# okieraised/rs-face-detection

Measured on NVIDIA B200. Metric: frames/s preproc+decode+NMS+align, higher is better.
Workload: dtype u8/f32

## Files before the change

rs_face_detection_b200/csrc/fd_align.cu:

```cuda
#include <algorithm>
#include <cmath>
#include <cstdio>
#include <cstdlib>
#include <vector>
#include <cfloat>
#include <type_traits>
#include "fd_internal.cuh"
#include "fd_estimate.cuh"
#include "fd_resize.cuh"

namespace fd {

struct EstArgs {
    const float *from;
    const float *to;
    const int *count_dev;
    int F;
    EstConst ec;
    double *M12;
    double *M_out;
    uint8_t *ok;
    uint8_t *ok_out;
};

// ... 335 lines not shown
    }
#pragma unroll
    for (int u = 0; u < N; ++u) {
        const int p = p0 + u * WARP_THREADS;
        unsigned lo0, hi0, lo1, hi1;
        extract6(q[u][0], q[u][1], off[u], lo0, hi0);
        extract6(q[u][2], q[u][3], off[u] + pitch, lo1, hi1);
        const unsigned v = blend24(lo0, hi0, lo1, hi1, axy[u] & 31, axy[u] >> 8);
        store_px(band_out, p, v, p < npix, packed);
    }
}

template <int FMT>
__device__ __forceinline__ void warp_round_border(const WarpItem &it, const int2 *__restrict__ dxy, const int2 *__restrict__ xy0, int cw,
                                                  unsigned cw_magic, int p0, int npix, uint8_t *band_out, bool packed) {
    const int p = min(p0, npix - 1);
    const int row = cw_magic ? (int)__umulhi((unsigned)p, cw_magic) : p, x = p - row * cw;
    const int2 d = dxy[x], r0 = xy0[row];
    const int X = (int)((unsigned)r0.x + (unsigned)d.x) >> 5, Y = (int)((unsigned)r0.y + (unsigned)d.y) >> 5;
    const unsigned v = FMT != SRC_BGR ? border_tap_blend_yuv<FMT>(it.data, it.pitch, it.uv, it.v, it.pitch_uv, it.w, it.h, X, Y)
                                      : border_tap_blend(it.data, it.w, it.h, it.pitch, it.lo_lim, it.hi_lim, X, Y);
    store_px(band_out, p0, v, p0 < npix, packed);
}

template <int FMT>
__global__ void __launch_bounds__(WARP_THREADS, 4) warp_kernel(WarpArgs a) {
    constexpr bool NV = FMT != SRC_BGR;
    extern __shared__ int2 wsm[];
    int2 *dxy = wsm;
    int2 *xy0 = dxy + a.cw;
    __shared__ int s_item[2];
    const int tid = threadIdx.x;
    pdl_wait();
    const int F = a.count_dev ? min(*a.count_dev, a.F) : a.F;
    const int n_items = F * a.bands;
    if (tid == 0) s_item[0] = atomicAdd(a.ticket, 1);
    __syncthreads();
    for (int par = 0;; par ^= 1) {
        const int item = s_item[par];
        if (item >= n_items) {
            pdl_trigger();
            break;
        }
        if (tid == 0) s_item[par ^ 1] = atomicAdd(a.ticket, 1);
        const int f = item / a.bands, band_y0 = (item - f * a.bands) * WARP_BAND;
        const int rows = min(WARP_BAND, a.ch - band_y0);
        const int npix = rows * a.cw;
        uint8_t *band_out = a.crops + ((size_t)f * a.ch + band_y0) * a.cw * 3;
        const bool packed = (reinterpret_cast<uintptr_t>(band_out) & 3) == 0 && (npix & 3) == 0;
        const FrameDev fr = a.frames[a.frame_idx ? a.frame_idx[f] : 0];
        if (!a.ok[f]) {
            int rx0 = 0, ry0 = 0;
            const bool valid = warp_fallback_roi(a, f, fr.w, fr.h, &rx0, &ry0);
            if (tid == 0 && band_y0 == 0 && a.mode_out) a.mode_out[f] = valid ? 2 : 0;
            if (valid) {
                const uint8_t *roi = fr.data + (size_t)ry0 * fr.pitch + (size_t)rx0 * 3;
                for (int p = tid; p < npix; p += WARP_THREADS) {
                    const int row = p / a.cw, x = p - row * a.cw;
                    const unsigned v = NV ? resize_pixel24_yuv<FMT>(fr.data, fr.pitch, fr.uv, fr.v_plane(), fr.pitch_uv, rx0, ry0, fr.w - rx0, fr.h - ry0, a.cw,
                                                                    a.ch, x, band_y0 + row)
                                          : resize_pixel24(roi, fr.pitch, fr.w - rx0, fr.h - ry0, a.cw, a.ch, x, band_y0 + row);
                    band_out[3 * p] = (uint8_t)v; band_out[3 * p + 1] = (uint8_t)(v >> 8); band_out[3 * p + 2] = (uint8_t)(v >> 16);
                }
            } else {
                for (int p = tid; p < npix * 3; p += WARP_THREADS) band_out[p] = 0;
            }
            __syncthreads();
            continue;
        }
        if (tid == 0 && band_y0 == 0 && a.mode_out) a.mode_out[f] = 1;
        const double *iM = a.M12 + (size_t)f * 12 + 6;
        const double i0 = iM[0], i1 = iM[1], i2 = iM[2], i3 = iM[3], i4 = iM[4], i5 = iM[5];
        for (int x = tid; x < a.cw; x += WARP_THREADS)
            dxy[x] = make_int2(__double2int_rn(i0 * x * 1024), __double2int_rn(i3 * x * 1024));
        if (tid >= WARP_THREADS - WARP_BAND) {
            const int r = tid - (WARP_THREADS - WARP_BAND), y = band_y0 + min(r, rows - 1);
// ... 88 lines not shown
template <int CW, int N, int FMT>
__device__ __forceinline__ void fixed_rounds_interior_yuv(const uint8_t *__restrict__ yp, unsigned py, const uint8_t *__restrict__ uvp,
                                                          const uint8_t *__restrict__ vp, unsigned puv, int2 d, const int2 *__restrict__ xy,
                                                          unsigned *__restrict__ outw, bool store, unsigned pack_sel) {
    YuvQuad<FMT> q[N];
    int axy[N];
#pragma unroll
    for (int u = 0; u < N; ++u) {
        const int2 r0 = xy[2 * u];
        const int X = (int)((unsigned)r0.x + (unsigned)d.x) >> 5, Y = (int)((unsigned)r0.y + (unsigned)d.y) >> 5;
        axy[u] = (X & 31) | ((Y & 31) << 14);
        yuv_quad_load<FMT>(yp, py, uvp, vp, puv, X >> 5, Y >> 5, q[u]);
    }
#pragma unroll
    for (int u = 0; u < N; ++u) {
        unsigned lo0, hi0, lo1, hi1;
        yuv_quad_taps<FMT>(q[u], lo0, hi0, lo1, hi1);
        const unsigned v = blend24_scaled(lo0, hi0, lo1, hi1, axy[u] & 31, axy[u] >> 8);
        const unsigned nv = __shfl_down_sync(0xffffffffu, v, 1);
        if (store) outw[u * (2 * CW * 3 / 4)] = __byte_perm(v, nv, pack_sel);
    }
}

template <int CW, int CH, int IR, int UN, int FMT>
__global__ void __launch_bounds__(2 * CW) warp_fixed_kernel(WarpArgs a) {
    constexpr bool NV = FMT != SRC_BGR;
    constexpr int T = 2 * CW, ITEMS = CH / IR, ROUNDS = IR / 2;
    static_assert(CH % IR == 0 && IR % 2 == 0 && T % 32 == 0 && (2 * CW * 3) % 4 == 0 && (IR * CW * 3) % 4 == 0, "fixed warp geometry");
    __shared__ int2 xy0[2][IR];
    __shared__ int s_item[2];
    const int tid = threadIdx.x;
    const int r = tid / CW, x = tid - r * CW;
    pdl_wait();
    const int F = a.count_dev ? min(*a.count_dev, a.F) : a.F;
    const int n_items = F * ITEMS;
    long long t_entry = 0, t_prev = 0, t_sum = 0;
    int n_done = 0;
    if (a.dbg && tid == 0) t_entry = warp_now();
    if (tid == 0) s_item[0] = atomicAdd(a.ticket, 1);
    __syncthreads();
    if (a.dbg && tid == 0) { t_prev = warp_now(); a.dbg[blockIdx.x * 8 + 1] = t_prev; }
    for (int par = 0;; par ^= 1) {
        const int item = s_item[par];
        if (a.dbg && tid == 0 && par == 1 && n_done == 1) a.dbg[blockIdx.x * 8 + 2] = warp_now();
        if (a.dbg && tid == 0) { const long long t = warp_now(); if (n_done) t_sum += t - t_prev; t_prev = t; ++n_done; }
        if (item >= n_items) {
            pdl_trigger();
            break;
        }
        if (tid == 0) s_item[par ^ 1] = atomicAdd(a.ticket, 1);
        const int f = item / ITEMS, y0 = (item - f * ITEMS) * IR;
        uint8_t *band_out = a.crops + ((size_t)f * CH + y0) * CW * 3;
        const bool okf = a.ok[f] != 0;
        const FrameDev *frp = a.frames + (a.frame_idx ? a.frame_idx[f] : 0);
        const uint8_t *data = frp->data;
        const int fw = frp->w, fh = frp->h, pitch = frp->pitch;
        const uint8_t *uvp = NV ? frp->uv : nullptr;
        const int pitch_uv = NV ? frp->pitch_uv : 0;
        const uint8_t *vp = nullptr;
        if constexpr (FMT == SRC_PLANAR) vp = frp->v_plane();
        int2 d = make_int2(0, 0);
        bool vote = true;
        if (okf) {
            const double *iM = a.M12 + (size_t)f * 12 + 6;
            const double i0 = iM[0], i3 = iM[3];
            d = make_int2(__double2int_rn(i0 * x * 1024), __double2int_rn(i3 * x * 1024));
            if (tid < IR || tid >= T - 4) {
                const double i1 = iM[1], i2 = iM[2], i4 = iM[4], i5 = iM[5];
                if (tid < IR) {
                    const int y = y0 + tid;
                    xy0[par][tid] = make_int2(__double2int_rn((i1 * y + i2) * 1024) + 16, __double2int_rn((i4 * y + i5) * 1024) + 16);
                } else {
                    const int c = tid - (T - 4), cx = (c & 1) ? CW - 1 : 0, y = y0 + ((c & 2) ? IR - 1 : 0);
                    const long long Xl = (long long)(__double2int_rn((i1 * y + i2) * 1024) + 16) + __double2int_rn(i0 * cx * 1024);
                    const long long Yl = (long long)(__double2int_rn((i4 * y + i5) * 1024) + 16) + __double2int_rn(i3 * cx * 1024);
                    const long long sx = Xl >> 10, sy = Yl >> 10;
                    vote = sx >= 0 && sx + 1 < fw && sy >= 0 && sy + 1 < fh - (NV ? 2 : 1);
                }
            }
        }
        const bool interior = __syncthreads_and(vote) && (NV ? yuv_interior_ok<FMT>(*frp)
                                                                 : (reinterpret_cast<uintptr_t>(data) & 7) == 0 && (pitch & 7) == 0 && pitch >= 16 &&
// ... 103 lines not shown
                    double *M12_dev, double *M_out_dev, uint8_t *ok_dev, uint8_t *ok_out_dev) {
    if (F_cap <= 0) return FD_OK;
    EstArgs a;
    a.from = from_dev;
    a.to = to_dev;
    a.count_dev = count_dev;
    a.F = F_cap;
    FD_TRY(make_est_const(ctx, &a.ec));
    a.M12 = M12_dev;
    a.M_out = M_out_dev;
    a.ok = ok_dev;
    a.ok_out = ok_out_dev;
    estimate_kernel<<<(F_cap * EST_LANES + 127) / 128, 128, 0, ctx->stream>>>(a);
    FD_LAUNCH_CHECK_NAMED(ctx, "estimate_kernel");
    return FD_OK;
}

int invert_launch(fd_ctx *ctx, const double *M_dev, int F, double *M12_dev, uint8_t *ok_dev) {
    if (F <= 0) return FD_OK;
    invert_kernel<<<(F + 127) / 128, 128, 0, ctx->stream>>>(M_dev, F, M12_dev, ok_dev);
    FD_LAUNCH_CHECK(ctx);
    return FD_OK;
}

template <int IR>
static void (*fixed_kernel_for(int fmt))(WarpArgs) {
    return fmt == SRC_NV12 ? warp_fixed_kernel<112, 112, IR, 4, SRC_NV12>
           : fmt == SRC_NV21 ? warp_fixed_kernel<112, 112, IR, 4, SRC_NV21>
           : fmt == SRC_PLANAR ? warp_fixed_kernel<112, 112, IR, 2, SRC_PLANAR> : warp_fixed_kernel<112, 112, IR, 4, SRC_BGR>;
}
static const char *const FIXED_NAMES[4] = {"warp_fixed_kernel", "warp_fixed_kernel_nv12", "warp_fixed_kernel_nv21", "warp_fixed_kernel_i420"};
static const char *const WARP_NAMES[4] = {"warp_kernel", "warp_kernel_nv12", "warp_kernel_nv21", "warp_kernel_i420"};

int warp_launch(fd_ctx *ctx, const FrameDev *frames_dev, const int32_t *frame_idx_dev, const double *M12_dev,
                const uint8_t *ok_dev, const int *count_dev, int F_cap, uint8_t *crops_dev, int cw, int ch, const WarpFallback &fb,
                int fmt) {
    if (F_cap <= 0) return FD_OK;
    WarpArgs a;
    a.bbox = fb.bbox;
    a.bbox_stride = fb.bbox_stride;
    a.sel = fb.sel;
    a.mode_out = fb.mode_out;
    a.frames = frames_dev;
    a.frame_idx = frame_idx_dev;
    a.M12 = M12_dev;
    a.ok = ok_dev;
    a.count_dev = count_dev;
    a.F = F_cap;
    a.crops = crops_dev;
    a.cw = cw;
    a.ch = ch;
    a.bands = (ch + WARP_BAND - 1) / WARP_BAND;
    a.cw_magic = cw > 1 ? (unsigned)((1ull << 32) / (unsigned)cw + 1ull) : 0u;
    FD_TRY(ticket_buffer(ctx));
    a.ticket = ctx->tickets.as<int>();
    a.dbg = nullptr;
    static const bool dbg_on = getenv("FD_WARP_DBG") != nullptr;
    static long long *dbg_dev = nullptr;
    if (dbg_on) {
        if (!dbg_dev) FD_CUDA(cudaMalloc(&dbg_dev, sizeof(long long) * 8 * 4096));
        FD_CUDA(cudaMemsetAsync(dbg_dev, 0, sizeof(long long) * 8 * 4096, ctx->stream));
        a.dbg = dbg_dev;
    }
    if (cw == 112 && ch == 112 && (reinterpret_cast<uintptr_t>(crops_dev) & 3) == 0) {
        static const int ir_env = getenv("FD_WARP_IR") ? atoi(getenv("FD_WARP_IR")) : 14;
        const int IR = ir_env == 16 ? 16 : 14;
        void (*kern)(WarpArgs) = IR == 16 ? fixed_kernel_for<16>(fmt) : fixed_kernel_for<14>(fmt);
        static int per_sm_fixed[4] = {0, 0, 0, 0};
        int &per_sm_k = per_sm_fixed[fmt];
        if (!per_sm_k) FD_CUDA(cudaOccupancyMaxActiveBlocksPerMultiprocessor(&per_sm_k, kern, 224, 0));
        const long long items = (long long)F_cap * (112 / IR);
        const int grid = (int)std::min<long long>(items, (long long)ctx->num_sms * std::max(per_sm_k, 1));
        FD_TRY(launch_pdl(ctx, kern, dim3(grid), dim3(224), 0, a));
        FD_LAUNCH_CHECK_NAMED(ctx, FIXED_NAMES[fmt]);
        if (dbg_on) {
            std::vector<long long> h(8 * (size_t)std::min(grid, 4096));
            cudaStreamSynchronize(ctx->stream);
            cudaMemcpy(h.data(), dbg_dev, sizeof(long long) * h.size(), cudaMemcpyDeviceToHost);
            long long t0 = h[0], t1 = h[3], first_sum = 0, item_sum = 0, items_n = 0, entry_max = h[0], tick_sum = 0;
            const int n = (int)h.size() / 8;
            for (int b = 0; b < n; ++b) {
                t0 = std::min(t0, h[8 * b]); t1 = std::max(t1, h[8 * b + 3]); entry_max = std::max(entry_max, h[8 * b]);
                tick_sum += h[8 * b + 1] - h[8 * b];
                if (h[8 * b + 2]) first_sum += h[8 * b + 2] - h[8 * b + 1];
                item_sum += h[8 * b + 5]; items_n += h[8 * b + 4];
            }
            fprintf(stderr, "[warp dbg] F=%d grid=%d span %.2f us; CTA entry spread %.2f us; first ticket %.2f us; first item %.2f us; mean item %.2f us over %lld items\n",
                    F_cap, grid, (t1 - t0) * 1e-3, (entry_max - t0) * 1e-3, tick_sum * 1e-3 / n, first_sum * 1e-3 / n, items_n ? item_sum * 1e-3 / items_n : 0.0, items_n);
        }
        return FD_OK;
    }
    const size_t smem = sizeof(int2) * ((size_t)cw + WARP_BAND);
    int per_sm = 0;
    void (*kern)(WarpArgs) = fmt == SRC_NV12 ? warp_kernel<SRC_NV12>
                             : fmt == SRC_NV21 ? warp_kernel<SRC_NV21>
                             : fmt == SRC_PLANAR ? warp_kernel<SRC_PLANAR> : warp_kernel<SRC_BGR>;
    FD_CUDA(cudaOccupancyMaxActiveBlocksPerMultiprocessor(&per_sm, kern, WARP_THREADS, smem));
    const long long items = (long long)F_cap * a.bands;
    const int grid = (int)std::min<long long>(items, (long long)ctx->num_sms * std::max(per_sm, 1));
    FD_TRY(launch_pdl(ctx, kern, dim3(grid), dim3(WARP_THREADS), smem, a));
    FD_LAUNCH_CHECK_NAMED(ctx, WARP_NAMES[fmt]);
    return FD_OK;
}

}
```

rs_face_detection_b200/csrc/fd_internal.cuh:

```cuda
#pragma once
#include <cuda_runtime.h>
#include <stdint.h>
#include <string>
#include <utility>
#include <vector>
#include "../../include/fd_b200.h"

#define FD_EXPORT extern "C" __attribute__((visibility("default")))

namespace fd {

void set_error(const std::string &msg);
int fail(int code, const std::string &msg);

#define FD_CUDA(call)                                                                                   \
    do {                                                                                                \
        cudaError_t _e = (call);                                                                        \
        if (_e != cudaSuccess)                                                                          \
            return ::fd::fail(FD_ERR_CUDA, std::string(#call) + ": " + cudaGetErrorString(_e));        \
    } while (0)
#define FD_TRY(call)                 \
    do {                             \
        int _s = (call);             \
        if (_s != FD_OK) return _s;  \
// ... 98 lines not shown
    int est_cap = 0;
    int align_cap_hint = 0;
    bool crowded = false;
    bool share_sms = false;
    bool est_valid = false;
    fd::DevBuf nms_ws[8];
    fd::DevBuf nms_ws_sp[4];
    fd::DevBuf pipe_frames;
    fd::DevBuf pipe_heads[3 * FD_MAX_STRIDES];
    fd::DevBuf pipe_tensor;
    fd::DevBuf pipe_crops;
    fd::DevBuf jpeg_coef, jpeg_planes, jpeg_frames, jpeg_desc;
    fd::DevBuf jpeg_raw;
    fd::DevBuf jpeg_stream, jpeg_aux;
    fd::DevBuf jpeg_sync, jpeg_flags;
    fd::PinnedBuf jpeg_coef_host, jpeg_desc_host, jpeg_aux_host, jpeg_flags_host;
    int jpeg_last_selfsync = 0, jpeg_last_rounds = 0;
    int64_t jpeg_last_h2d = 0;
    int jpeg_last_B = 0;
    int jpeg_last_gpu_entropy = 0;
    fd::DevBuf pipe_mode;
    int last_B = 0;
    int last_out_cap = 0;
    bool last_fused = false;
    bool detect_pending = false;
    float last_iou = 0.f;
    std::vector<unsigned char> frames_shadow;
    std::vector<float> det_scale_shadow;
    bool align_replay = false;
    uint8_t *align_crops = nullptr;
    int align_cap = 0;
    double *align_M_out = nullptr;
    uint8_t *align_ok_out = nullptr;
};

namespace fd {

int check_ctx(const fd_ctx *ctx);

void trace_mark(fd_ctx *ctx, const char *file, int line, const char *name);
#define FD_LAUNCH_CHECK_NAMED(ctx, name)                                          \
    do {                                                                          \
        (ctx)->launches++;                                                        \
        FD_CUDA(cudaGetLastError());                                              \
        if ((ctx)->trace_on) ::fd::trace_mark((ctx), __FILE__, __LINE__, (name)); \
    } while (0)
#define FD_LAUNCH_CHECK(ctx) FD_LAUNCH_CHECK_NAMED(ctx, nullptr)

template <typename... KArgs, typename... Args>
int launch_pdl(fd_ctx *ctx, void (*kern)(KArgs...), dim3 grid, dim3 block, size_t smem, Args &&...args) {
    cudaLaunchConfig_t cfg = {};
    cfg.gridDim = grid;
    cfg.blockDim = block;
    cfg.dynamicSmemBytes = smem;
    cfg.stream = ctx->stream;
    cudaLaunchAttribute attr[1];
    attr[0].id = cudaLaunchAttributeProgrammaticStreamSerialization;
    attr[0].val.programmaticStreamSerializationAllowed = ctx->share_sms ? 0 : 1;
    cfg.attrs = attr;
    cfg.numAttrs = 1;
    FD_CUDA(cudaLaunchKernelEx(&cfg, kern, std::forward<Args>(args)...));
    return FD_OK;
}

#ifdef __CUDACC__

__device__ __forceinline__ void pdl_wait() { asm volatile("griddepcontrol.wait;" ::: "memory"); }
__device__ __forceinline__ void pdl_trigger() { asm volatile("griddepcontrol.launch_dependents;" ::: "memory"); }

__device__ __forceinline__ uint32_t desc_key(float f) {
    uint32_t u = (f == 0.0f) ? 0u : __float_as_uint(f);
    uint32_t asc = (u & 0x80000000u) ? ~u : (u | 0x80000000u);
    return ~asc;
}

__device__ __forceinline__ float box_area(float4 b) {
// ... 75 lines not shown
```

rs_face_detection_b200/csrc/fd_pipeline.cu:

```cuda
#include <algorithm>
#include <cmath>
#include <climits>
#include <cstdlib>
#include <cstddef>
#include <cstring>
#include "fd_internal.cuh"

namespace fd {

static int wait_stream(fd_ctx *ctx) {
    if (ctx->blocking_sync && ctx->ev_block) {
        FD_CUDA(cudaEventRecord(ctx->ev_block, ctx->stream));
        FD_CUDA(cudaEventSynchronize(ctx->ev_block));
    } else {
        FD_CUDA(cudaStreamSynchronize(ctx->stream));
    }
    return FD_OK;
}

static void letterbox(int h, int w, int size_w, int size_h, int *new_w, int *new_h, float *det_scale) {
    volatile float im_ratio = (float)h / (float)w;
    volatile float model_ratio = (float)size_h / (float)size_w;
    if (im_ratio > model_ratio) {
        *new_h = size_h;
// ... 70 lines not shown
    fl->yuv = frames;
    fl->layout = layout;
    return FD_OK;
}

static int upload_frame_table(fd_ctx *ctx, FrameList frames, int B, float *det_scale_host, int *max_row_bytes) {
    const int fmt = frames.yuv ? yuv420_format(frames.layout) : SRC_BGR;
    std::vector<FrameDev> tab(B);
    int mrb = 0;
    for (int i = 0; i < B; ++i) {
        float ds;
        memset(&tab[i], 0, sizeof(FrameDev));
        if (frames.yuv) {
            const int w = frames.yuv[i].width;
            FD_TRY(fill_frame_yuv420(ctx, frames.yuv[i], frames.layout, &tab[i], &ds));
            mrb = std::max(mrb, fmt == SRC_PLANAR ? 2 * ((w / 2 + 15) & ~15) : w);
        } else {
            FD_REQUIRE(frames.bgr[i].data != nullptr, "frame: null data");
            FD_TRY(fill_frame(ctx, frames.bgr[i], frames.bgr[i].data, &tab[i], &ds));
            mrb = std::max(mrb, frames.bgr[i].width * 3);
        }
        if (det_scale_host) det_scale_host[i] = ds;
    }
    if (max_row_bytes) *max_row_bytes = mrb;
    ctx->frames_fmt = fmt;
    const size_t bytes = sizeof(FrameDev) * (size_t)B;
    if (ctx->frames_shadow.size() == bytes && memcmp(ctx->frames_shadow.data(), tab.data(), bytes) == 0) return FD_OK;
    FD_TRY(ctx->pinned[0].reserve(bytes));
    FD_TRY(ctx->frames_dev.reserve(bytes));
    FD_CUDA(cudaEventSynchronize(ctx->ev[0]));
    memcpy(ctx->pinned[0].p, tab.data(), bytes);
    FD_CUDA(cudaMemcpyAsync(ctx->frames_dev.p, ctx->pinned[0].p, bytes, cudaMemcpyHostToDevice, ctx->stream));
    FD_CUDA(cudaEventRecord(ctx->ev[0], ctx->stream));
    ctx->frames_shadow.assign(reinterpret_cast<unsigned char *>(tab.data()), reinterpret_cast<unsigned char *>(tab.data()) + bytes);
    return FD_OK;
}

static int align_enqueue(fd_ctx *ctx, const float *lmk_dev, const int32_t *frame_idx_dev,
                         const int *count_dev, int F_cap, uint8_t *crops_dev, double *M_dev, uint8_t *ok_dev, bool from_detect,
                         WarpFallback fb) {
    if (F_cap <= 0) return FD_OK;
    ctx->align_cap_hint = std::max(ctx->align_cap_hint, F_cap);
    const bool reuse = from_detect && ctx->est_valid && F_cap <= ctx->est_cap && !M_dev;
    if (!reuse) {
        ctx->est_valid = false;
        FD_TRY(ctx->align_M.reserve(sizeof(double) * 12 * (size_t)F_cap));
        FD_TRY(ctx->align_ok.reserve((size_t)F_cap));
        FD_TRY(estimate_launch(ctx, lmk_dev, nullptr, count_dev, F_cap, ctx->align_M.as<double>(), M_dev, ctx->align_ok.as<uint8_t>(), nullptr));
    }
    fb.mode_out = ok_dev;
    FD_TRY(warp_launch(ctx, ctx->frames_dev.as<FrameDev>(), frame_idx_dev, ctx->align_M.as<double>(), ctx->align_ok.as<uint8_t>(), count_dev,
                       F_cap, crops_dev, ctx->cfg.crop_w, ctx->cfg.crop_h, fb, ctx->frames_fmt));
    return FD_OK;
}

static WarpFallback detect_fallback(fd_ctx *ctx) {
    WarpFallback fb;
    fb.bbox = ctx->out_det.as<float>();
    fb.bbox_stride = 5;
    return fb;
}

static int detect_resolve(fd_ctx *ctx) {
    if (!ctx->detect_pending) return FD_OK;
    const int B = ctx->last_B;
    int st[4] = {0, 0, 0, 0};
// ... 910 lines not shown
```

rs_face_detection_b200/csrc/fd_preprocess.cu:

```cuda
#include <algorithm>
#include "fd_internal.cuh"
#include "fd_resize.cuh"

namespace fd {

constexpr int PRE_ROWS = 8;

struct PreArgs {
    const FrameDev *frames;
    float *out;
    int out_w, out_h;
    float pixel_scale, means[3], stds[3];
    int row_buf_bytes;
    int vec_store;
};

__device__ __forceinline__ const uint8_t *stage_row(uint8_t *buf, const uint8_t *__restrict__ src, int nbytes) {
    const int mis = (int)(reinterpret_cast<uintptr_t>(src) & 15);
    uint8_t *dst = buf + mis;
    const int head = mis ? min(nbytes, 16 - mis) : 0;
    for (int i = threadIdx.x; i < head; i += blockDim.x) dst[i] = __ldg(src + i);
    const int nvec = (nbytes - head) >> 4;
    const int4 *s4 = reinterpret_cast<const int4 *>(src + head);
    int4 *d4 = reinterpret_cast<int4 *>(dst + head);
    for (int v = threadIdx.x; v < nvec; v += blockDim.x) d4[v] = __ldg(s4 + v);
    const int done = head + (nvec << 4);
    for (int i = done + threadIdx.x; i < nbytes; i += blockDim.x) dst[i] = __ldg(src + i);
    return dst;
}

template <int FMT>
__global__ void preprocess_kernel(PreArgs a) {
    constexpr bool NV = FMT != SRC_BGR, PL = FMT == SRC_PLANAR;
    extern __shared__ __align__(16) unsigned char smem[];
    const int ow = a.out_w;
    float *lut = reinterpret_cast<float *>(smem);
    int *xo0 = reinterpret_cast<int *>(lut + 768);
    int *xo1 = xo0 + ow;
    short *xa0 = reinterpret_cast<short *>(xo1 + ow);
    short *xa1 = xa0 + ow;
    size_t tab_bytes = 768 * 4 + (size_t)ow * 12;
    tab_bytes = (tab_bytes + 15) & ~(size_t)15;
    uint8_t *rowbuf0 = smem + tab_bytes;
    uint8_t *rowbuf1 = rowbuf0 + a.row_buf_bytes;
    uint8_t *rowbuf2 = rowbuf1 + a.row_buf_bytes, *rowbuf3 = rowbuf2 + a.row_buf_bytes;
    const int half = a.row_buf_bytes >> 1;

    for (int i = threadIdx.x; i < 768; i += blockDim.x) {
        int c = i >> 8, v = i & 255;
        lut[i] = __fdiv_rn(__fsub_rn(__fdiv_rn((float)v, a.pixel_scale), a.means[c]), a.stds[c]);
    }
    pdl_wait();
    const FrameDev f = a.frames[blockIdx.y];
    for (int x = threadIdx.x; x < f.new_w; x += blockDim.x) {
        x_taps(x, f.scale_x, f.w, &xo0[x], &xo1[x], &xa0[x], &xa1[x]);
        if (NV) { xo0[x] /= 3; xo1[x] /= 3; }
    }
    __syncthreads();
    const float pad_r = lut[2 * 256], pad_g = lut[1 * 256], pad_b = lut[0];
    const size_t plane = (size_t)a.out_h * ow;
    float *out_img = a.out + (size_t)blockIdx.y * 3 * plane;
    const int ngroups = (ow + 3) >> 2;
    const int row_begin = blockIdx.x * PRE_ROWS;
    const int row_end = min(row_begin + PRE_ROWS, a.out_h);
    const int src_row_bytes = NV ? f.w : f.w * 3;

    for (int dy = row_begin; dy < row_end; ++dy) {
        float *o_r = out_img + (size_t)dy * ow;
        float *o_g = o_r + plane;
        float *o_b = o_g + plane;
        const bool content = dy < f.new_h;
        const uint8_t *r0 = nullptr, *r1 = nullptr, *c0 = nullptr, *c1 = nullptr, *v0 = nullptr, *v1 = nullptr;
        int b0 = 0, b1 = 0;
        if (content) {
            int y0, y1;
            y_taps(dy, f.scale_y, f.h, &y0, &y1, &b0, &b1);
            r0 = stage_row(rowbuf0, f.data + (size_t)y0 * f.pitch, src_row_bytes);
            r1 = b1 != 0 ? stage_row(rowbuf1, f.data + (size_t)y1 * f.pitch, src_row_bytes) : r0;
            if (PL) {
                const int cb = f.w >> 1;
                const size_t oc0 = (size_t)(y0 >> 1) * f.pitch_uv, oc1 = (size_t)(y1 >> 1) * f.pitch_uv;
                c0 = stage_row(rowbuf2, f.uv + oc0, cb);
                v0 = stage_row(rowbuf2 + half, f.v_plane() + oc0, cb);
                const bool two = b1 != 0 && (y1 >> 1) != (y0 >> 1);
                c1 = two ? stage_row(rowbuf3, f.uv + oc1, cb) : c0;
// ... 11 lines not shown
                const int x = 4 * g + j;
                if (content && x < f.new_w) {
                    const int x0 = xo0[x], x1 = xo1[x], a0 = xa0[x], a1 = xa1[x];
                    if (NV) {
                        const unsigned p = resize_px24(yuv_px24<FMT>(r0, c0, v0, x0), yuv_px24<FMT>(r0, c0, v0, x1),
                                                       b1 != 0 ? yuv_px24<FMT>(r1, c1, v1, x0) : 0u, b1 != 0 ? yuv_px24<FMT>(r1, c1, v1, x1) : 0u,
                                                       a0, a1, b0, b1);
                        vb[j] = lut[p & 255u];
                        vg[j] = lut[256 + ((p >> 8) & 255u)];
                        vr[j] = lut[512 + (p >> 16)];
                    } else {
                        vb[j] = lut[resize_px(r0, r1, x0, x1, a0, a1, b0, b1)];
                        vg[j] = lut[256 + resize_px(r0, r1, x0 + 1, x1 + 1, a0, a1, b0, b1)];
                        vr[j] = lut[512 + resize_px(r0, r1, x0 + 2, x1 + 2, a0, a1, b0, b1)];
                    }
                } else {
                    vb[j] = pad_b; vg[j] = pad_g; vr[j] = pad_r;
                }
            }
            if (a.vec_store) {
                *reinterpret_cast<float4 *>(o_r + 4 * g) = make_float4(vr[0], vr[1], vr[2], vr[3]);
                *reinterpret_cast<float4 *>(o_g + 4 * g) = make_float4(vg[0], vg[1], vg[2], vg[3]);
                *reinterpret_cast<float4 *>(o_b + 4 * g) = make_float4(vb[0], vb[1], vb[2], vb[3]);
            } else {
                for (int j = 0; j < 4 && 4 * g + j < ow; ++j) {
                    o_r[4 * g + j] = vr[j];
                    o_g[4 * g + j] = vg[j];
                    o_b[4 * g + j] = vb[j];
                }
            }
        }
        if (content) __syncthreads();
    }
}

constexpr int PRE2_STAGES = 4;
constexpr int PRE2_ROWS = 16;

__device__ __forceinline__ uint32_t smem_u32(const void *p) { return (uint32_t)__cvta_generic_to_shared(p); }
__device__ __forceinline__ void mbar_init(uint64_t *bar, int count) {
    asm volatile("mbarrier.init.shared::cta.b64 [%0], %1;" ::"r"(smem_u32(bar)), "r"(count));
}
__device__ __forceinline__ void mbar_expect_tx(uint64_t *bar, uint32_t bytes) {
    asm volatile("mbarrier.arrive.expect_tx.shared::cta.b64 _, [%0], %1;" ::"r"(smem_u32(bar)), "r"(bytes) : "memory");
}
__device__ __forceinline__ void mbar_wait(uint64_t *bar, uint32_t parity) {
    asm volatile(
        "{\n\t.reg .pred p;\n\t"
        "WAIT_%=:\n\t"
        "mbarrier.try_wait.parity.shared::cta.b64 p, [%0], %1;\n\t"
        "@p bra DONE_%=;\n\t"
        "bra WAIT_%=;\n\t"
        "DONE_%=:\n\t}" ::"r"(smem_u32(bar)), "r"(parity) : "memory");
}
__device__ __forceinline__ void bulk_g2s(void *dst_smem, const void *src_gmem, uint32_t bytes, uint64_t *bar) {
    asm volatile("cp.async.bulk.shared::cluster.global.mbarrier::complete_tx::bytes [%0], [%1], %2, [%3];" ::"r"(smem_u32(dst_smem)),
                 "l"(src_gmem), "r"(bytes), "r"(smem_u32(bar))
                 : "memory");
}

template <bool IDENT, int FMT>
__global__ void __launch_bounds__(256) preprocess_tma_kernel(PreArgs a) {
    constexpr bool NV = FMT != SRC_BGR, PL = FMT == SRC_PLANAR;
    constexpr int SLOTS = NV ? 4 : 2;
    extern __shared__ __align__(128) unsigned char smem[];
    uint64_t *full = reinterpret_cast<uint64_t *>(smem);
    float *lut = reinterpret_cast<float *>(smem + 64);
    uint8_t *bufs = smem + 64 + 3072;
    const int tid = threadIdx.x;
    const int ow = a.out_w;
    const int rb = a.row_buf_bytes;

    if (tid == 0) {
#pragma unroll
        for (int s = 0; s < PRE2_STAGES; ++s) mbar_init(&full[s], 1);
        asm volatile("fence.mbarrier_init.release.cluster;" ::: "memory");
    }
    if (!IDENT) {
        for (int i = tid; i < 768; i += blockDim.x) {
            int c = i >> 8, v = i & 255;
            lut[i] = __fdiv_rn(__fsub_rn(__fdiv_rn((float)v, a.pixel_scale), a.means[c]), a.stds[c]);
        }
    }
    pdl_wait();
    const FrameDev f = a.frames[blockIdx.y];
    int x0[4];
    short wa0[4], wa1[4];
    bool point = true;
#pragma unroll
    for (int j = 0; j < 4; ++j) {
        const int x = 4 * tid + j;
        x0[j] = -1;
        wa0[j] = 0;
        wa1[j] = 0;
        if (x < f.new_w) {
            int o1;
            x_taps(x, f.scale_x, f.w, &x0[j], &o1, &wa0[j], &wa1[j]);
            if (NV) x0[j] /= 3;
            point &= (wa1[j] == 0);
        }
    }
    const bool hpoint = __syncthreads_and(point);

    const float pad_b = IDENT ? 0.0f : lut[0], pad_g = IDENT ? 0.0f : lut[256], pad_r = IDENT ? 0.0f : lut[512];
    const size_t plane = (size_t)a.out_h * ow;
    float *out_img = a.out + (size_t)blockIdx.y * 3 * plane;
    const int row_begin = blockIdx.x * PRE2_ROWS;
    const int row_end = min(row_begin + PRE2_ROWS, a.out_h);
    const int n_content = max(0, min(f.new_h, row_end) - row_begin);
    const uint32_t copy_bytes = (uint32_t)(((NV ? f.w : f.w * 3) + 15) & ~15);
    const uint32_t half_bytes = (uint32_t)(((f.w >> 1) + 15) & ~15);
    const int half = rb >> 1;
    const bool active = 4 * tid < ow;

    auto issue = [&](int it) {
        int y0, y1, b0, b1;
        y_taps(row_begin + it, f.scale_y, f.h, &y0, &y1, &b0, &b1);
// ... 63 lines not shown
                                                           b1 != 0 ? yuv_px24<FMT>(r1, c1, v1, o0) : 0u,
                                                           b1 != 0 ? yuv_px24<FMT>(r1, c1, v1, o1) : 0u, q0, q1, b0, b1);
                            pb = p & 255u; pg = (p >> 8) & 255u; pr = p >> 16;
                        } else {
                            pb = resize_px(r0, r1, o0, o1, q0, q1, b0, b1);
                            pg = resize_px(r0, r1, o0 + 1, o1 + 1, q0, q1, b0, b1);
                            pr = resize_px(r0, r1, o0 + 2, o1 + 2, q0, q1, b0, b1);
                        }
                        vb[j] = IDENT ? (float)pb : lut[pb];
                        vg[j] = IDENT ? (float)pg : lut[256 + pg];
                        vr[j] = IDENT ? (float)pr : lut[512 + pr];
                    } else {
                        vb[j] = pad_b; vg[j] = pad_g; vr[j] = pad_r;
                    }
                }
            }
            float *o_r = out_img + (size_t)dy * ow + 4 * tid;
            __stcs(reinterpret_cast<float4 *>(o_r), make_float4(vr[0], vr[1], vr[2], vr[3]));
            __stcs(reinterpret_cast<float4 *>(o_r + plane), make_float4(vg[0], vg[1], vg[2], vg[3]));
            __stcs(reinterpret_cast<float4 *>(o_r + 2 * plane), make_float4(vb[0], vb[1], vb[2], vb[3]));
        }
        __syncthreads();
    }
    if (active) {
        const float4 zr = make_float4(pad_r, pad_r, pad_r, pad_r), zg = make_float4(pad_g, pad_g, pad_g, pad_g),
                     zb = make_float4(pad_b, pad_b, pad_b, pad_b);
        for (int dy = row_begin + n_content; dy < row_end; ++dy) {
            float *o_r = out_img + (size_t)dy * ow + 4 * tid;
            __stcs(reinterpret_cast<float4 *>(o_r), zr);
            __stcs(reinterpret_cast<float4 *>(o_r + plane), zg);
            __stcs(reinterpret_cast<float4 *>(o_r + 2 * plane), zb);
        }
    }
}

__global__ void resize_u8_kernel(FrameDev f, uint8_t *__restrict__ out, int out_h, int out_w) {
    const int dy = blockIdx.y;
    int y0, y1, b0, b1;
    y_taps(dy, f.scale_y, f.h, &y0, &y1, &b0, &b1);
    const uint8_t *r0 = f.data + (size_t)y0 * f.pitch, *r1 = f.data + (size_t)y1 * f.pitch;
    for (int x = blockIdx.x * blockDim.x + threadIdx.x; x < out_w; x += gridDim.x * blockDim.x) {
        int x0, x1;
        short a0, a1;
        x_taps(x, f.scale_x, f.w, &x0, &x1, &a0, &a1);
        uint8_t *o = out + ((size_t)dy * out_w + x) * 3;
        if (f.h == out_h && f.w == out_w) {
            o[0] = r0[x * 3]; o[1] = r0[x * 3 + 1]; o[2] = r0[x * 3 + 2];
        } else {
            o[0] = (uint8_t)resize_px(r0, r1, x0, x1, a0, a1, b0, b1);
            o[1] = (uint8_t)resize_px(r0, r1, x0 + 1, x1 + 1, a0, a1, b0, b1);
            o[2] = (uint8_t)resize_px(r0, r1, x0 + 2, x1 + 2, a0, a1, b0, b1);
        }
    }
}

struct CropArgs {
    const uint8_t *crops;
    const int *count_dev;
    int F, in_h, in_w, out_h, out_w;
    float mean[3], mul[3];
    float *out;
};
__global__ void __launch_bounds__(256) crops_to_tensor_kernel(CropArgs a) {
    const int F = a.count_dev ? min(*a.count_dev, a.F) : a.F;
    const int groups_per_row = (a.out_w + 3) >> 2;
    const int groups = a.out_h * groups_per_row;
// ... 35 lines not shown
            }
        }
    }
}

int crops_to_tensor_launch(fd_ctx *ctx, const uint8_t *crops_dev, const int *count_dev, int F, int in_h, int in_w, int out_h,
                           int out_w, const float *mean_rgb, const float *mul_rgb, float *out_dev) {
    if (F <= 0) return FD_OK;
    CropArgs a;
    a.crops = crops_dev;
    a.count_dev = count_dev;
    a.F = F; a.in_h = in_h; a.in_w = in_w; a.out_h = out_h; a.out_w = out_w;
    for (int i = 0; i < 3; ++i) { a.mean[i] = mean_rgb[i]; a.mul[i] = mul_rgb[i]; }
    a.out = out_dev;
    const int groups = out_h * ((out_w + 3) / 4);
    dim3 grid(std::max(1, std::min(16, (groups + 255) / 256)), std::min(F, 65535));
    if (count_dev) grid.y = std::min(F, std::max(1, ctx->num_sms * 8 / (int)grid.x));
    crops_to_tensor_kernel<<<grid, 256, 0, ctx->stream>>>(a);
    FD_LAUNCH_CHECK_NAMED(ctx, "crops_to_tensor_kernel");
    return FD_OK;
}

static const char *const TMA_NAMES[4] = {"preprocess_tma_kernel", "preprocess_tma_kernel_nv12", "preprocess_tma_kernel_nv21",
                                         "preprocess_tma_kernel_i420"};
static const char *const PRE_NAMES[4] = {"preprocess_kernel", "preprocess_kernel_nv12", "preprocess_kernel_nv21", "preprocess_kernel_i420"};

template <bool IDENT>
static void (*tma_kernel_for(int fmt))(PreArgs) {
    return fmt == SRC_NV12 ? preprocess_tma_kernel<IDENT, SRC_NV12>
           : fmt == SRC_NV21 ? preprocess_tma_kernel<IDENT, SRC_NV21>
           : fmt == SRC_PLANAR ? preprocess_tma_kernel<IDENT, SRC_PLANAR> : preprocess_tma_kernel<IDENT, SRC_BGR>;
}

int preprocess_launch(fd_ctx *ctx, const FrameDev *frames_dev, int B, float *out_nchw_dev, int max_row_bytes, bool rows_aligned16,
                      int fmt) {
    constexpr int SLOTS_NV = 4;
    const bool nv = fmt != SRC_BGR;
    PreArgs a;
    a.frames = frames_dev;
    a.out = out_nchw_dev;
    a.out_w = ctx->cfg.image_w;
    a.out_h = ctx->cfg.image_h;
    a.pixel_scale = ctx->cfg.pixel_scale;
    bool ident = a.pixel_scale == 1.0f;
    for (int i = 0; i < 3; ++i) {
        a.means[i] = ctx->cfg.pixel_means[i];
        a.stds[i] = ctx->cfg.pixel_stds[i];
        ident = ident && a.means[i] == 0.0f && a.stds[i] == 1.0f;
    }
    a.row_buf_bytes = ((max_row_bytes + 32) + 15) & ~15;
    a.vec_store = (a.out_w % 4 == 0) && ((reinterpret_cast<uintptr_t>(out_nchw_dev) & 15) == 0);
    const int ngroups = (a.out_w + 3) / 4;
    if (rows_aligned16 && a.vec_store && ngroups <= 256) {
        a.row_buf_bytes = (max_row_bytes + 15) & ~15;
        size_t smem = 64 + 3072 + (size_t)PRE2_STAGES * (nv ? SLOTS_NV : 2) * a.row_buf_bytes;
        if (smem <= (size_t)ctx->max_smem_optin) {
            int threads = std::max(32, ((ngroups + 31) / 32) * 32);
            dim3 grid((a.out_h + PRE2_ROWS - 1) / PRE2_ROWS, B);
            void (*kern)(PreArgs) = ident ? tma_kernel_for<true>(fmt) : tma_kernel_for<false>(fmt);
            FD_CUDA(cudaFuncSetAttribute(kern, cudaFuncAttributeMaxDynamicSharedMemorySize, (int)smem));
            FD_TRY(launch_pdl(ctx, kern, grid, dim3(threads), smem, a));
            FD_LAUNCH_CHECK_NAMED(ctx, TMA_NAMES[fmt]);
            return FD_OK;
        }
    }
    size_t tab_bytes = 768 * 4 + (size_t)a.out_w * 12;
    tab_bytes = (tab_bytes + 15) & ~(size_t)15;
    size_t smem = tab_bytes + (nv ? SLOTS_NV : 2) * (size_t)a.row_buf_bytes;
    if (smem > (size_t)ctx->max_smem_optin) return fail(FD_ERR_INVALID, "fd_preprocess: source row too wide for shared-memory staging");
    void (*kern)(PreArgs) = fmt == SRC_NV12 ? preprocess_kernel<SRC_NV12>
                            : fmt == SRC_NV21 ? preprocess_kernel<SRC_NV21>
                            : fmt == SRC_PLANAR ? preprocess_kernel<SRC_PLANAR> : preprocess_kernel<SRC_BGR>;
    FD_CUDA(cudaFuncSetAttribute(kern, cudaFuncAttributeMaxDynamicSharedMemorySize, (int)smem));
    int threads = std::min(1024, std::max(64, ((ngroups + 31) / 32) * 32));
    dim3 grid((a.out_h + PRE_ROWS - 1) / PRE_ROWS, B);
    FD_TRY(launch_pdl(ctx, kern, grid, dim3(threads), smem, a));
    FD_LAUNCH_CHECK_NAMED(ctx, PRE_NAMES[fmt]);
    return FD_OK;
}

int resize_launch(fd_ctx *ctx, const FrameDev &frame, uint8_t *out_dev, int out_h, int out_w) {
    dim3 grid(std::max(1, std::min(64, (out_w + 127) / 128)), out_h);
    resize_u8_kernel<<<grid, 128, 0, ctx->stream>>>(frame, out_dev, out_h, out_w);
    FD_LAUNCH_CHECK(ctx);
// ... 5 lines not shown
```

Baseline: 355,000.

## Overlap preprocess with preceding warp kernel via early PDL trigger and range checks

Result: faster. 360,700, median of 6 (+1.6%).

```diff
diff --git a/rs_face_detection_b200/csrc/fd_align.cu b/rs_face_detection_b200/csrc/fd_align.cu
--- a/rs_face_detection_b200/csrc/fd_align.cu
+++ b/rs_face_detection_b200/csrc/fd_align.cu
@@ -391,16 +391,14 @@
     __shared__ int s_item[2];
     const int tid = threadIdx.x;
     pdl_wait();
+    pdl_trigger();
     const int F = a.count_dev ? min(*a.count_dev, a.F) : a.F;
     const int n_items = F * a.bands;
     if (tid == 0) s_item[0] = atomicAdd(a.ticket, 1);
     __syncthreads();
     for (int par = 0;; par ^= 1) {
         const int item = s_item[par];
-        if (item >= n_items) {
-            pdl_trigger();
-            break;
-        }
+        if (item >= n_items) break;
         if (tid == 0) s_item[par ^ 1] = atomicAdd(a.ticket, 1);
         const int f = item / a.bands, band_y0 = (item - f * a.bands) * WARP_BAND;
         const int rows = min(WARP_BAND, a.ch - band_y0);
@@ -555,6 +553,7 @@
     const int tid = threadIdx.x;
     const int r = tid / CW, x = tid - r * CW;
     pdl_wait();
+    pdl_trigger();
     const int F = a.count_dev ? min(*a.count_dev, a.F) : a.F;
     const int n_items = F * ITEMS;
     long long t_entry = 0, t_prev = 0, t_sum = 0;
@@ -567,10 +566,7 @@
         const int item = s_item[par];
         if (a.dbg && tid == 0 && par == 1 && n_done == 1) a.dbg[blockIdx.x * 8 + 2] = warp_now();
         if (a.dbg && tid == 0) { const long long t = warp_now(); if (n_done) t_sum += t - t_prev; t_prev = t; ++n_done; }
-        if (item >= n_items) {
-            pdl_trigger();
-            break;
-        }
+        if (item >= n_items) break;
         if (tid == 0) s_item[par ^ 1] = atomicAdd(a.ticket, 1);
         const int f = item / ITEMS, y0 = (item - f * ITEMS) * IR;
         uint8_t *band_out = a.crops + ((size_t)f * CH + y0) * CW * 3;
@@ -740,6 +736,25 @@
 static const char *const FIXED_NAMES[4] = {"warp_fixed_kernel", "warp_fixed_kernel_nv12", "warp_fixed_kernel_nv21", "warp_fixed_kernel_i420"};
 static const char *const WARP_NAMES[4] = {"warp_kernel", "warp_kernel_nv12", "warp_kernel_nv21", "warp_kernel_i420"};
 
+static void note_warp(fd_ctx *ctx, const WarpArgs &a) {
+    if (a.frames != ctx->frames_dev.as<FrameDev>() || a.sel) return;
+    const size_t F = (size_t)a.F;
+    auto add = [&](const void *p, size_t n) {
+        if (p) ctx->warp_ranges.emplace_back(reinterpret_cast<uintptr_t>(p), reinterpret_cast<uintptr_t>(p) + n);
+    };
+    ctx->warp_ranges.clear();
+    add(a.crops, F * a.ch * a.cw * 3);
+    add(a.mode_out, F);
+    add(a.frames, ctx->frames_shadow.size());
+    add(a.frame_idx, F * sizeof(int));
+    add(a.M12, F * 12 * sizeof(double));
+    add(a.ok, F);
+    add(a.count_dev, sizeof(int));
+    add(a.bbox, F * a.bbox_stride * sizeof(float));
+    add(a.ticket, 2 * sizeof(int));
+    ctx->after_warp = true;
+}
+
 int warp_launch(fd_ctx *ctx, const FrameDev *frames_dev, const int32_t *frame_idx_dev, const double *M12_dev,
                 const uint8_t *ok_dev, const int *count_dev, int F_cap, uint8_t *crops_dev, int cw, int ch, const WarpFallback &fb,
                 int fmt) {
@@ -778,9 +793,11 @@
         int &per_sm_k = per_sm_fixed[fmt];
         if (!per_sm_k) FD_CUDA(cudaOccupancyMaxActiveBlocksPerMultiprocessor(&per_sm_k, kern, 224, 0));
         const long long items = (long long)F_cap * (112 / IR);
-        const int grid = (int)std::min<long long>(items, (long long)ctx->num_sms * std::max(per_sm_k, 1));
+        constexpr int FIXED_CTAS_PER_SM = 4;
+        const int grid = (int)std::min<long long>(items, (long long)ctx->num_sms * std::max(std::min(per_sm_k, FIXED_CTAS_PER_SM), 1));
         FD_TRY(launch_pdl(ctx, kern, dim3(grid), dim3(224), 0, a));
         FD_LAUNCH_CHECK_NAMED(ctx, FIXED_NAMES[fmt]);
+        note_warp(ctx, a);
         if (dbg_on) {
             std::vector<long long> h(8 * (size_t)std::min(grid, 4096));
             cudaStreamSynchronize(ctx->stream);
@@ -808,6 +825,7 @@
     const int grid = (int)std::min<long long>(items, (long long)ctx->num_sms * std::max(per_sm, 1));
     FD_TRY(launch_pdl(ctx, kern, dim3(grid), dim3(WARP_THREADS), smem, a));
     FD_LAUNCH_CHECK_NAMED(ctx, WARP_NAMES[fmt]);
+    note_warp(ctx, a);
     return FD_OK;
 }
 
diff --git a/rs_face_detection_b200/csrc/fd_internal.cuh b/rs_face_detection_b200/csrc/fd_internal.cuh
--- a/rs_face_detection_b200/csrc/fd_internal.cuh
+++ b/rs_face_detection_b200/csrc/fd_internal.cuh
@@ -154,6 +154,8 @@
     int align_cap = 0;
     double *align_M_out = nullptr;
     uint8_t *align_ok_out = nullptr;
+    bool after_warp = false;
+    std::vector<std::pair<uintptr_t, uintptr_t>> warp_ranges;
 };
 
 namespace fd {
@@ -164,6 +166,7 @@
 #define FD_LAUNCH_CHECK_NAMED(ctx, name)                                          \
     do {                                                                          \
         (ctx)->launches++;                                                        \
+        (ctx)->after_warp = false;                                                \
         FD_CUDA(cudaGetLastError());                                              \
         if ((ctx)->trace_on) ::fd::trace_mark((ctx), __FILE__, __LINE__, (name)); \
     } while (0)
diff --git a/rs_face_detection_b200/csrc/fd_pipeline.cu b/rs_face_detection_b200/csrc/fd_pipeline.cu
--- a/rs_face_detection_b200/csrc/fd_pipeline.cu
+++ b/rs_face_detection_b200/csrc/fd_pipeline.cu
@@ -126,6 +126,7 @@
     memcpy(ctx->pinned[0].p, tab.data(), bytes);
     FD_CUDA(cudaMemcpyAsync(ctx->frames_dev.p, ctx->pinned[0].p, bytes, cudaMemcpyHostToDevice, ctx->stream));
     FD_CUDA(cudaEventRecord(ctx->ev[0], ctx->stream));
+    ctx->after_warp = false;
     ctx->frames_shadow.assign(reinterpret_cast<unsigned char *>(tab.data()), reinterpret_cast<unsigned char *>(tab.data()) + bytes);
     return FD_OK;
 }
diff --git a/rs_face_detection_b200/csrc/fd_preprocess.cu b/rs_face_detection_b200/csrc/fd_preprocess.cu
--- a/rs_face_detection_b200/csrc/fd_preprocess.cu
+++ b/rs_face_detection_b200/csrc/fd_preprocess.cu
@@ -13,7 +13,12 @@
     float pixel_scale, means[3], stds[3];
     int row_buf_bytes;
     int vec_store;
+    int indep;
 };
+
+__device__ __forceinline__ void pdl_wait_if_last(const PreArgs &a) {
+    if (a.indep && threadIdx.x == 0 && blockIdx.x == gridDim.x - 1 && blockIdx.y == gridDim.y - 1) pdl_wait();
+}
 
 __device__ __forceinline__ const uint8_t *stage_row(uint8_t *buf, const uint8_t *__restrict__ src, int nbytes) {
     const int mis = (int)(reinterpret_cast<uintptr_t>(src) & 15);
@@ -50,7 +55,7 @@
         int c = i >> 8, v = i & 255;
         lut[i] = __fdiv_rn(__fsub_rn(__fdiv_rn((float)v, a.pixel_scale), a.means[c]), a.stds[c]);
     }
-    pdl_wait();
+    if (!a.indep) pdl_wait();
     const FrameDev f = a.frames[blockIdx.y];
     for (int x = threadIdx.x; x < f.new_w; x += blockDim.x) {
         x_taps(x, f.scale_x, f.w, &xo0[x], &xo1[x], &xa0[x], &xa1[x]);
@@ -128,6 +133,7 @@
         }
         if (content) __syncthreads();
     }
+    pdl_wait_if_last(a);
 }
 
 constexpr int PRE2_STAGES = 4;
@@ -178,7 +184,7 @@
             lut[i] = __fdiv_rn(__fsub_rn(__fdiv_rn((float)v, a.pixel_scale), a.means[c]), a.stds[c]);
         }
     }
-    pdl_wait();
+    if (!a.indep) pdl_wait();
     const FrameDev f = a.frames[blockIdx.y];
     int x0[4];
     short wa0[4], wa1[4];
@@ -308,6 +314,7 @@
             __stcs(reinterpret_cast<float4 *>(o_r + 2 * plane), zb);
         }
     }
+    pdl_wait_if_last(a);
 }
 
 __global__ void resize_u8_kernel(FrameDev f, uint8_t *__restrict__ out, int out_h, int out_w) {
@@ -409,6 +416,30 @@
            : fmt == SRC_PLANAR ? preprocess_tma_kernel<IDENT, SRC_PLANAR> : preprocess_tma_kernel<IDENT, SRC_BGR>;
 }
 
+static bool beside_warp(const fd_ctx *ctx, const FrameDev *frames_dev, const float *out, size_t bytes) {
+    if (!ctx->after_warp || ctx->share_sms || frames_dev != ctx->frames_dev.as<FrameDev>()) return false;
+    using Range = std::pair<uintptr_t, uintptr_t>;
+    auto overlap = [](const Range &a, const Range &b) { return a.first < b.second && b.first < a.second; };
+    std::vector<Range> planes;
+    auto add = [&](const uint8_t *p, size_t n) { planes.emplace_back(reinterpret_cast<uintptr_t>(p), reinterpret_cast<uintptr_t>(p) + n); };
+    const FrameDev *tab = reinterpret_cast<const FrameDev *>(ctx->frames_shadow.data());
+    for (size_t i = 0; i < ctx->frames_shadow.size() / sizeof(FrameDev); ++i) {
+        const FrameDev &f = tab[i];
+        add(f.data, (size_t)f.h * f.pitch);
+        if (f.uv) add(f.uv, (size_t)(f.h / 2) * f.pitch_uv);
+        if (f.uv && f.v_off) add(f.v_plane(), (size_t)(f.h / 2) * f.pitch_uv);
+    }
+    const Range t(reinterpret_cast<uintptr_t>(out), reinterpret_cast<uintptr_t>(out) + bytes);
+    for (const Range &w : ctx->warp_ranges) {
+        if (overlap(t, w)) return false;
+        for (const Range &p : planes)
+            if (overlap(p, w)) return false;
+    }
+    for (const Range &p : planes)
+        if (overlap(t, p)) return false;
+    return true;
+}
+
 int preprocess_launch(fd_ctx *ctx, const FrameDev *frames_dev, int B, float *out_nchw_dev, int max_row_bytes, bool rows_aligned16,
                       int fmt) {
     constexpr int SLOTS_NV = 4;
@@ -427,6 +458,7 @@
     }
     a.row_buf_bytes = ((max_row_bytes + 32) + 15) & ~15;
     a.vec_store = (a.out_w % 4 == 0) && ((reinterpret_cast<uintptr_t>(out_nchw_dev) & 15) == 0);
+    a.indep = beside_warp(ctx, frames_dev, out_nchw_dev, sizeof(float) * 3 * (size_t)a.out_h * a.out_w * B);
     const int ngroups = (a.out_w + 3) / 4;
     if (rows_aligned16 && a.vec_store && ngroups <= 256) {
         a.row_buf_bytes = (max_row_bytes + 15) & ~15;
```
